# satoken/ractip

Hardware: AMD Instinct MI355X
Metric: sequence-pairs/sec (incl. bp+hp+ap DP; host strings in, thresholded matrices out) at n=500 (higher is better)
Workload: dtype f64; 1 GPU; synthetic random pairs n=500/500, std::mt19937(12345) stream (BASELINE config 3); scoring=CONTRAfold complementary (708 weights)

## Files before the change

### ractip_amd/csrc/ctx.h

```cpp
#pragma once
#include <hip/hip_runtime.h>

#include <cassert>
#include <cstdint>
#include <cstring>
#include <string>
#include <type_traits>
#include <vector>

#include "../../include/ractip_hot.h"
#include "batch.h"
#include "batch_request.h"
#include "local_windows.h"
#include "score_model.h"
#include "lin_model.h"
#include "vienna_model.h"
#include "scale_order.h"
#include "span_fold.h"

struct rh_ctx;

namespace rh::host {

struct DevBuf {
// ... 18 lines not shown
        return hipMemcpy(p, host, cap, hipMemcpyHostToDevice);
    }
};

struct LocalHp {
    LocalDuplex2Plan D;
    int windowed = 0;
    bool valid = false;
    DevBuf hp, logz;
    int tile[2] = {0, 0};
    double ms[2] = {0, 0};
};

struct LinSet {
    LinModel h;
    DevObj<LinModel> d;
    DevObj<double> wT;
};

struct VLinSet {
    VLinModel* h = nullptr;
    DevObj<VLinModel> d;
    ~VLinSet() { delete h; }
};

struct GraphSlot {
    hipGraphExec_t exec = nullptr;
    size_t key = 0;
    int launches = 0, far = 0;
};

struct SweepPlan {
    enum Org { kNone, kStrips, kPairs, kLookahead, kDiagonals, kDxStrip8, kDxSweep4, kDxSweepW };
    enum Far { kFarNone, kFarLds, kFarGather, kFarPacked };
    Org org = kNone;
    int W = 0;
    int BS = 0;
    int filt = 0;
    Far far = kFarNone;
    int far2_from = 0;
    int banded = 0;
    int repack2 = 0;
    const char* fine = "";
    const char* far_name = "";
};

static_assert(std::has_unique_object_representations_v<SweepPlan> && std::has_unique_object_representations_v<McBatch>);
static_assert(sizeof(DxLinBatch) == 4 * sizeof(void*) + 6 * sizeof(int) + 3 * sizeof(size_t) + 16 * sizeof(double), "no padding");

struct McLinArgs {
    McBatch B;
    const LinSet* lin;
    double* logz;
    int* bad;
    SweepPlan plan;
    const int* small_list;
    const int* n_sweep;
    const int* n_short;
    SweepPlan plan_sweep, plan_short;
    int routed, n_small, nmax_sweep, short_count, nmax_short;
    int phase, pin, strip_xcd;
    int f5_pass, f5_jlo;
    int up_w, pad_;
    McLinArgs() { std::memset(this, 0, sizeof *this); }
};

struct McVlinArgs {
// ... 81 lines not shown
    DevObj<DxLinModel> d_dxlin_r[4];
    DxLinModel h_dxlin_r[4];
    std::vector<int> rescaled_dx;
    DxLinBatch dxl = {};
    size_t dxl_layout = 0;
    size_t dx_bytes = 0;
    bool dxtab_log = false;
    int co_seed = 1;
    int dx_strip = 1;
    int dx_quad = 1;
    int dx_w = 4;
    int last_dx_path = 0;
    int far_mfma = 1;
    int lookahead = 2;
    int strip = 3;
    int far2 = -1;
    int strip_w = 8;
    int small_on = 0;
    std::vector<int> small_list;
    DevBuf d_small_list;
    DevBuf d_n_sweep;
    int nmax_sweep = 0;
    DevBuf d_n_short;
    int n_short = 0, nmax_short = 0;
    int strip_filt = 1;
    bool strip_filt_ok = false;
    int co_cut_min = 0, co_cut_max = 0;
    int co_window = 1;
    int acc_final_t = 1;
    int acc_wide = 1;
    int strip_xcd = 1;
    int f5_pass = 1;
    int far_pk = 1;
    int use_graphs = 1;
    GraphSlot g_in, g_out, g_dx;
    int mode = RH_MODE_AUTO;
    int duplex_mode = RH_MODE_INHERIT;
    int lin_w = 4;
    int lin_w_in = 4;
    int lin_bs = 16;
    int last_path = 0;
    bool last_went_log = false;
    SweepPlan plan[3];
    int max_w = 1;
    int region_acc = 0;
    DevBuf d_acc;
    hipEvent_t acc_ev[2] = {nullptr, nullptr};
    bool acc_timed = false;

    int np = 0, ns = 0;
    std::vector<int> pair_seq;
    std::vector<int> pair_seq_dev;
    bool indexed = false;
    bool has_mc = false, has_dx = false, computed = false;
    std::vector<int> n;
    McBatch mc = {};
    DxBatch dx = {};
    DevBuf d_seq;
    DevBuf d_n;
    DevBuf d_pseq;
    DevBuf d_pn;
    DevBuf d_pidx;
    DevBuf d_mctab;
    DevBuf d_corowp;
    DevBuf d_rowp;
    DevBuf d_pk;
// ... 160 lines not shown
```

### ractip_amd/csrc/kernels.h

```cpp
#pragma once
#include <hip/hip_runtime.h>

#include "../../include/ractip_hot.h"
#include "batch.h"
#include "score_model.h"
#include "lin_model.h"
#include "vienna_model.h"

namespace rh {
__global__ void mc_init(McBatch B);
__global__ void mc_inside_diag(McBatch B, const ScoreModel* __restrict__ M, int d, int pin);
__global__ void mc_outside_diag(McBatch B, const ScoreModel* __restrict__ M, int d, int pin);
__global__ void mc_unpaired(McBatch B, int max_w);
struct AccArgs {
    const LinModel* lin;
    const ScoreModel* score;
    double* scratch;
    int max_w, pad_;
};
constexpr int kAccTile = 64, kAccK = 16;
constexpr size_t acc_scratch_doubles(int ld) { return 3 * (size_t)ld * ld + 2 * 31 * (size_t)ld; }
template <int PATH> __global__ void cf_acc_hrows(McBatch B, AccArgs A);
template <int PATH> __global__ void cf_acc_hcols(McBatch B, AccArgs A);
template <int PATH> __global__ void cf_acc_gaps(McBatch B, AccArgs A);
template <int PATH> __global__ void cf_acc_final(McBatch B, AccArgs A);
template <int PATH> __global__ void cf_acc_sbuild(McBatch B, AccArgs A);
template <int PATH> __global__ void cf_acc_seed(McBatch B, AccArgs A);
template <int PATH> __global__ void cf_acc_link(McBatch B, AccArgs A, int flip);
template <int PATH> __global__ void cf_acc_close(McBatch B, AccArgs A, int j, int flip);
__global__ void dx_sweep_diag(DxBatch B, const ScoreModel* __restrict__ M, int t);
__global__ void dx_logz(DxBatch B, const ScoreModel* __restrict__ M);
__global__ void dx_posterior(DxBatch B);
__global__ void dx_hp_clear_rest(DxBatch B);
__global__ void lin_init(McBatch B, const LinModel* __restrict__ L, int* __restrict__ bad);
template <int W, int BS, int MODE> __global__ void lin_inside_diag(McBatch B, const LinModel* __restrict__ L, int d, double lam_d, int pin);
template <int W, int BS> __global__ void lin_outside_diag(McBatch B, const LinModel* __restrict__ L, int d, int pin, int* __restrict__ bad);
template <int W, int BS> __global__ void lin_outside_pair(McBatch B, const LinModel* __restrict__ L, int d, int khi, int pin, int* __restrict__ bad);
template <int BS> __global__ void lin_far_inside(McBatch B, int D);
template <int BS> __global__ void lin_far_outside(McBatch B, int D);
__global__ void lin_far_inside_mfma(McBatch B, int D);
__global__ void lin_far_outside_mfma(McBatch B, int D);
template <int SWEEP> __global__ void lin_pack_tiles(McBatch B, int Dblk, int outside, int banded);
template <int KD, int W, int FILT> __global__ void lin_inside_strip(McBatch B, const LinModel* __restrict__ L, const double* __restrict__ wT, int d0, double lam_d0, int pin);
template <int KD, int W, int FILT> __global__ void lin_outside_strip(McBatch B, const LinModel* __restrict__ L, const double* __restrict__ wT, int d0, int pin, int* __restrict__ bad);
__global__ void lin_f5i_tail(McBatch B, const LinModel* __restrict__ L, int jlo);
__global__ void lin_f5i_pass(McBatch B, const LinModel* __restrict__ L, int jlo);
void launch_lin_small(const McBatch& B, const LinModel* L, const double* wpad, const int* list, int nlist, int* bad, hipStream_t stream);
__global__ void lin_f5o_head(McBatch B, const LinModel* __restrict__ L, int khi, int klo);
__global__ void lin_f5o_pass(McBatch B, const LinModel* __restrict__ L);
__global__ void lin_far_inside_pk(McBatch B, int D, int l2);
__global__ void lin_far_outside_pk(McBatch B, int D, int l2);
__global__ void lin_far2_inside(McBatch B, int D2, int l2);
__global__ void lin_far2_outside(McBatch B, int D2, int l2);
__global__ void lin_finish(McBatch B, const LinModel* __restrict__ L, double* __restrict__ logz, int* __restrict__ bad);
template <int W> __global__ void dxl_sweep(DxLinBatch B, const DxLinModel* __restrict__ L, int step, int groups);
__global__ void dxl_sweep4(DxLinBatch B, const DxLinModel* __restrict__ L, int step, int groups);
__global__ void dxl_strip8(DxLinBatch B, const DxLinModel* __restrict__ L, int step);
template <bool S20> __global__ void dxvl_sweep4(DxLinBatch B, const VLinModel* __restrict__ L, const VDxLin* __restrict__ D, int step);
template <bool S20> __global__ void dxvl_logz_part(DxLinBatch B, const VLinModel* __restrict__ L, const VDxLin* __restrict__ D, double* __restrict__ zpart,
                               int* __restrict__ cpart, int nchunk);
__global__ void dxvl_logz_final(DxLinBatch B, double s, const double* __restrict__ zpart, const int* __restrict__ cpart, int nchunk,
                                double* __restrict__ zbar, double* __restrict__ logz, int* __restrict__ bad);
constexpr int kLzThreads = 256;
size_t dxl_logz_lds_bytes(int lds);
__global__ void dxl_logz_part(DxLinBatch B, const DxLinModel* __restrict__ L, double* __restrict__ zpart, int* __restrict__ cpart, int nchunk);
__global__ void dxl_logz_final(DxLinBatch B, const DxLinModel* __restrict__ L, const double* __restrict__ zpart, const int* __restrict__ cpart, int nchunk,
                               double* __restrict__ zbar, double* __restrict__ logz, int* __restrict__ bad);
__global__ void dxl_posterior(DxLinBatch B, const double* __restrict__ zbar, int* __restrict__ bad);
__global__ void dxv_sweep_diag(DxBatch B, const ViennaDx* __restrict__ V, int t);
__global__ void dxv_logz(DxBatch B, const ViennaDx* __restrict__ V);
__global__ void dxv_posterior(DxBatch B);
__global__ void mcv_init(McBatch B);
__global__ void mcv_inside_diag(McBatch B, const ViennaDx* __restrict__ V, int d, int pin);
__global__ void mcv_outside_diag(McBatch B, const ViennaDx* __restrict__ V, int d, int pin);
__global__ void mcv_acc_prep(McBatch B, const ViennaDx* __restrict__ V);
__global__ void mcv_acc_hscan(McBatch B, int slot);
__global__ void vlin_acc_prep(McBatch B, const VLinModel* __restrict__ L, const double* __restrict__ hplen);
__global__ void vlin_acc_gaps(McBatch B, const VLinModel* __restrict__ L, double* __restrict__ gaps, int ng, int nchunk, double* __restrict__ part);
__global__ void vlin_acc_gsum(McBatch B, double* __restrict__ gaps, const double* __restrict__ part, int ng, int nchunk);
__global__ void vlin_acc_gaps_wide(McBatch B, const VLinModel* __restrict__ L, double* __restrict__ gaps);
__global__ void vlin_acc_final_t(McBatch B, const VLinModel* __restrict__ L, const double* __restrict__ gaps, int max_w);
__global__ void vlin_acc_hsum(McBatch B, int max_w);
__global__ void vlin_acc_gsuf(McBatch B, double* __restrict__ gaps);
__global__ void vlin_acc_final(McBatch B, const VLinModel* __restrict__ L, const double* __restrict__ gaps, int max_w);
// ... 64 lines not shown
```

### ractip_amd/csrc/launch_contrafold.hip

```cpp
#include <hip/hip_runtime.h>

#include <algorithm>
#include <cmath>
#include <cstring>
#include <string>
#include <vector>

#include "ctx.h"
#include "f5_stage.h"
#include "kernels.h"

__global__ void log_finish(rh::McBatch B, double* __restrict__ logz)
{
    const int sq = blockIdx.x * blockDim.x + threadIdx.x;
    if (sq < B.ns) logz[sq] = B.f5i[(size_t)sq * B.ld + B.n[sq]];
}

namespace rh::host {

int launch_mc_log(rh_ctx* c, int pin, const McBatch& B, double* logz_out)
{
    hipLaunchKernelGGL(mc_init, dim3((B.ns + 63) / 64), dim3(64), 0, c->s_mc, B);
    for (int d = 0; d <= B.nmax - 1; d++) {
        const int waves = std::max(B.nmax - 1 - d, 0) + 1;
        KLAUNCH(c, 0, mc_inside_diag, pin ? dim3(B.ns, (waves + 3) / 4) : dim3((waves + 3) / 4, B.ns), dim3(256), c->s_mc, B, c->d_model, d, pin);
        c->n_launch[0]++;
    }
    HIP_TRY(c, hipEventRecord(c->ev[kEvMcInside], c->s_mc));
    for (int d = B.nmax - 2; d >= 0; d--) {
        const int waves = (B.nmax - 1 - d) + 1;
        KLAUNCH(c, 2, mc_outside_diag, pin ? dim3(B.ns, (waves + 3) / 4) : dim3((waves + 3) / 4, B.ns), dim3(256), c->s_mc, B, c->d_model, d, pin);
        c->n_launch[1]++;
    }
    hipLaunchKernelGGL(log_finish, dim3((B.ns + 63) / 64), dim3(64), 0, c->s_mc, B, logz_out);
    hipLaunchKernelGGL(mc_unpaired, dim3((B.nmax + 63) / 64, B.ns), dim3(256), 0, c->s_mc, B, c->max_w);
    return RH_OK;
}

template <int PATH>
static void acc_kernels(const McBatch& B, const AccArgs& A, hipStream_t st)
{
    const int n = B.nmax, ns = B.ns, w = A.max_w;
    hipLaunchKernelGGL(cf_acc_hrows<PATH>, dim3((n + 255) / 256, ns), dim3(256), 0, st, B, A);
// ... 19 lines not shown
    A.lin = lin ? (const LinModel*)lin->d : nullptr;
    A.score = c->d_model;
    A.scratch = c->d_acc.as<double>();
    A.max_w = c->max_w;
    if (timed) {
        for (auto& e : c->acc_ev) if (!e) HIP_TRY(c, hipEventCreate(&e));
        HIP_TRY(c, hipEventRecord(c->acc_ev[0], c->s_mc));
    }
    if (lin) acc_kernels<0>(B, A, c->s_mc);
    else acc_kernels<1>(B, A, c->s_mc);
    HIP_TRY(c, hipGetLastError());
    if (timed) {
        HIP_TRY(c, hipEventRecord(c->acc_ev[1], c->s_mc));
        c->acc_timed = true;
    }
    return RH_OK;
}

using InsideDiagK = void (*)(McBatch, const LinModel*, int, double, int);
struct DiagKernels { int W, BS; Named<InsideDiagK> in; Named<decltype(&lin_outside_diag<4, 16>)> out; };
#define DIAG(W, BS) {W, BS, NAMED(lin_inside_diag<W, BS, 0>), NAMED(lin_outside_diag<W, BS>)}
const DiagKernels kDiag[] = {DIAG(8, 0), DIAG(16, 0), DIAG(4, 16), DIAG(8, 16), DIAG(16, 16), DIAG(8, 32), DIAG(16, 32)};
const Named<InsideDiagK> kInsidePair = NAMED(lin_inside_diag<4, 16, 3>);
const Named<InsideDiagK> kInsideAhead[2] = {NAMED(lin_inside_diag<4, 16, 1>), NAMED(lin_inside_diag<4, 16, 2>)};
struct PairKernels { int W; Named<decltype(&lin_outside_pair<4, 16>)> out; };
const PairKernels kOutsidePair[] = {{4, NAMED(lin_outside_pair<4, 16>)}, {8, NAMED(lin_outside_pair<8, 16>)}};
struct StripKernels { int W, filt; Named<decltype(&lin_inside_strip<8, 4, 0>)> in; Named<decltype(&lin_outside_strip<8, 4, 0>)> out; };
#define STRIP(W, FILT) {W, FILT, NAMED(lin_inside_strip<8, W, FILT>), NAMED(lin_outside_strip<8, W, FILT>)}
const StripKernels kStrip[] = {STRIP(4, 0), STRIP(8, 1), STRIP(8, 0)};
struct LdsKernels { int BS; Named<decltype(&lin_far_inside<16>)> in, out; };
const LdsKernels kLds[] = {{16, NAMED(lin_far_inside<16>), NAMED(lin_far_outside<16>)}, {32, NAMED(lin_far_inside<32>), NAMED(lin_far_outside<32>)}};
const Named<decltype(&lin_far_inside_mfma)> kFarGather[2] = {NAMED(lin_far_inside_mfma), NAMED(lin_far_outside_mfma)};
const Named<decltype(&lin_far_inside_pk)> kFarPacked[2] = {NAMED(lin_far_inside_pk), NAMED(lin_far_outside_pk)};
#undef DIAG
#undef STRIP
static const DiagKernels& diag_kernels(int W, int BS) { return row_of(kDiag, [&](const DiagKernels& r) { return r.W == W && r.BS == BS; }); }
static const PairKernels& pair_kernels(int W) { return row_of(kOutsidePair, [&](const PairKernels& r) { return r.W == W; }); }
static const StripKernels& strip_kernels(int W, int filt) { return row_of(kStrip, [&](const StripKernels& r) { return r.W == W && r.filt == filt; }); }
static const LdsKernels& lds_kernels(int BS) { return row_of(kLds, [&](const LdsKernels& r) { return r.BS == BS; }); }

const char* far_name(SweepPlan::Far far, int BS, int phase)
{
    switch (far) {
        case SweepPlan::kFarLds: return phase == 0 ? lds_kernels(BS).in.name : lds_kernels(BS).out.name;
        case SweepPlan::kFarGather: return kFarGather[phase].name;
        case SweepPlan::kFarPacked: return kFarPacked[phase].name;
        default: return "";
    }
}
void far_products(const rh_ctx* c, int phase, int nmax, bool mfma, SweepPlan* P)
{
    const int from = c->far2 >= 0 ? (c->far2 ? 1 : 0) : 384;
    P->far = P->BS == 0 ? SweepPlan::kFarNone : !mfma ? SweepPlan::kFarLds : c->far_pk ? SweepPlan::kFarPacked : SweepPlan::kFarGather;
    P->far2_from = P->far == SweepPlan::kFarPacked && from > 0 && nmax >= from ? from : 0;
    P->far_name = far_name(P->far, P->BS, phase);
}

void far_inside_after(const SweepPass& S, int done)
{
    rh_ctx* c = S.c;
    const McBatch& B = S.B;
    const int D = S.P.BS ? done / S.P.BS + 1 : 0, last_block = S.last_block(), l2 = S.P.far2_from;
    if (S.P.BS == 0 || done % S.P.BS != 0 || D < 4 || D > last_block) return;
    if (S.P.far == SweepPlan::kFarLds) KLAUNCH(c, 1, (lds_kernels(S.P.BS).in.kern), dim3(last_block - D + 1, B.ns), dim3(256), S.st, B, D);
    else if (S.P.far == SweepPlan::kFarGather) KLAUNCH(c, 1, (kFarGather[0].kern), dim3(last_block - D + 1, B.ns), dim3(256), S.st, B, D);
    else {
        KLAUNCH(c, 1, lin_pack_tiles<0>, dim3(B.nb - (D - 2), B.ns, 2), dim3(256), S.st, B, D - 2, 0, (int)S.P.banded);
        if (l2 && (D + 3) % 4 == 0) {
            const int D2 = (D + 3) / 4, last2 = (B.nmax - 1) / 64;
            if (D2 >= 4 && D2 <= last2) KLAUNCH(c, 1, lin_far2_inside, dim3(last2 - D2 + 1, B.ns), dim3(256), S.st, B, D2, l2);
        }
        KLAUNCH(c, 1, (kFarPacked[0].kern), dim3(last_block - D + 1, B.ns), dim3(256), S.st, B, D, l2);
    }
    c->n_launch[S.k]++;
    c->n_far[S.k]++;
}
void far_outside_before(SweepPass& S, int d)
{
    rh_ctx* c = S.c;
    const McBatch& B = S.B;
    const int D = S.P.BS ? (d + 1) / S.P.BS - 1 : 0, last_block = S.last_block(), l2 = S.P.far2_from;
    if (S.P.BS == 0 || (d + 1) % S.P.BS != 0 || D < 0 || D > last_block) return;
    if (S.P.far == SweepPlan::kFarLds) KLAUNCH(c, 3, (lds_kernels(S.P.BS).out.kern), dim3(last_block - D + 1, B.ns, 2), dim3(256), S.st, B, D);
    else if (S.P.far == SweepPlan::kFarGather) KLAUNCH(c, 3, (kFarGather[1].kern), dim3(last_block - D + 1, B.ns, 2), dim3(256), S.st, B, D);
    else {
        if (D + 2 <= last_block) KLAUNCH(c, 3, lin_pack_tiles<1>, dim3(B.nb - (D + 2), B.ns, 1), dim3(256), S.st, B, D + 2, 1, 0);
        if (l2) {
            const int last2 = (B.nmax - 1) / 64;
            for (; S.far2_next >= 0 && 4 * S.far2_next + 3 >= D; S.far2_next--)
                KLAUNCH(c, 3, lin_far2_outside, dim3(last2 - S.far2_next + 1, B.ns, 2), dim3(256), S.st, B, S.far2_next, l2);
        }
        KLAUNCH(c, 3, (kFarPacked[1].kern), dim3(last_block - D + 1, B.ns, 2), dim3(256), S.st, B, D, l2);
    }
    c->n_launch[S.k]++;
    c->n_far[S.k]++;
}
void far_outside_begin(SweepPass& S, int top)
{
    if (S.P.BS == 0) return;
    rh_ctx* c = S.c;
    const McBatch& B = S.B;
    const int last_block = S.last_block(), banded = S.P.banded;
    if (S.P.far == SweepPlan::kFarPacked) {
        S.far2_next = (B.nmax - 1) / 64;
        if (S.P.repack2 && last_block - 1 > 2) KLAUNCH(c, 3, lin_pack_tiles<1>, dim3(B.nb - 2, B.ns, 2), dim3(256), S.st, B, 2, 0, banded);
        for (int Dblk = std::max(2, last_block - 1); Dblk <= last_block; Dblk++)
            KLAUNCH(c, 3, lin_pack_tiles<1>, dim3(B.nb - Dblk, B.ns, 2), dim3(256), S.st, B, Dblk, 0, banded);
    }
    for (int d = (last_block + 1) * S.P.BS - 1; d > top; d -= S.P.BS) far_outside_before(S, d);
}

SweepPlan plan_mc_lin(const rh_ctx* c, int phase, int nmax)
{
    SweepPlan P;
    const int w = phase == 0 ? c->lin_w_in : c->lin_w;
    P.BS = c->lin_bs == 0 || c->lin_bs == 32 ? c->lin_bs : 16;
    P.W = w == 16 ? 16 : (w == 4 && P.BS == 16 ? 4 : 8);
    const bool all_orgs = P.W == 4 && P.BS == 16, strips_ok = c->far_pk && c->far_mfma && c->lin_bs == 16 && nmax >= kStripMinN;
    const bool strips_on = (c->strip & (phase == 0 ? 1 : 2)) && strips_ok, strips = all_orgs && strips_on;
    const StripKernels& strip = strip_kernels(c->strip_w, c->strip_w == 8 && c->strip_filt && c->strip_filt_ok);
    const DiagKernels& diag = diag_kernels(P.W, P.BS);
    bool mfma = P.BS == 16 && c->far_mfma;
    P.org = SweepPlan::kDiagonals;
    P.fine = phase == 0 ? diag.in.name : diag.out.name;
    if (strips) {
        P.org = SweepPlan::kStrips;
        P.W = strip.W;
        P.filt = strip.filt;
    } else if (phase == 0 && all_orgs && c->lookahead == 2) {
        P.org = SweepPlan::kPairs;
        P.fine = kInsidePair.name;
        mfma = true;
    } else if (phase == 0 && all_orgs && c->lookahead) {
        P.org = SweepPlan::kLookahead;
        P.fine = kInsideAhead[0].name;
    } else if (phase == 1 && mfma && (P.W == 4 || P.W == 8) && c->lookahead == 2) {
        P.org = SweepPlan::kPairs;
        P.fine = pair_kernels(P.W).out.name;
    }
    far_products(c, phase, nmax, mfma, &P);
// ... 171 lines not shown
```

### ractip_amd/csrc/mccaskill_far.hip

```cpp
#include <hip/hip_runtime.h>

#include "batch.h"
#include "lin_model.h"
#include "kernels.h"

namespace rh {

static_assert((int)VL_FM1 == (int)L_FM1 && (int)VL_FM == (int)L_FM && (int)VL_FM2O == (int)L_FM2O && (int)VL_FM2F == (int)L_FM2F &&
                  (int)VL_FMOF == (int)L_FMOF && (int)VL_FM1OF == (int)L_FM1OF,
              "LinTable and VLinTable disagree on a slot of the block products: FM1, FM, FM2O, FM2F, FMOF, FM1OF");

namespace {

__device__ __forceinline__ double cellv(const double* __restrict__ T, int ld, int n, int x, int y)
{
    return (x >= 1 && x <= y && y <= n - 1) ? T[(size_t)(y - x) * ld + x] : 0.0;
}

template <int BS, bool TR>
__device__ __forceinline__ void load_chunk(double (*dst)[BS + 1], const double* __restrict__ T, int ld, int n, int x0, int y0)
{
    const int u = threadIdx.x % BS;
    constexpr int DPP = 256 / BS;
    for (int dd = threadIdx.x / BS; dd < 2 * BS - 1; dd += DPP) {
        const int v = u + dd - (BS - 1);
        if (v >= 0 && v < BS) {
            const double val = cellv(T, ld, n, x0 + u, y0 + v);
            if (TR) dst[v][u] = val; else dst[u][v] = val;
        }
    }
}

template <int BS>
struct Acc {
    static constexpr int R = BS / 16;
    double c[R][R];
    __device__ __forceinline__ void zero()
// ... 158 lines not shown
__global__ __launch_bounds__(256) void lin_far_outside_mfma(McBatch B, int D)
{
    __shared__ double A[4][16][17], Bm[4][16][17], red[4][256];
    const int sq = blockIdx.y;
    const int n = B.n[sq];
    const int I = blockIdx.x, J = I + D;
    if (J * 16 > n - 1) return;
    const int w = threadIdx.x >> 6;
    const int ld = B.ld;
    double* __restrict__ tab = B.tab + (size_t)sq * B.seq_stride;
    const double* __restrict__ fm1 = tab + (size_t)L_FM1 * B.tab_stride;
    const double* __restrict__ fm = tab + (size_t)L_FM * B.tab_stride;
    const double* __restrict__ fm2o = tab + (size_t)L_FM2O * B.tab_stride;
    d4 acc = {0.0, 0.0, 0.0, 0.0};
    if (blockIdx.z == 0) {
        for (int K = w; K <= I - 2; K += 4) {
            load_chunk16_wave<true>(A[w], fm1, ld, n, K * 16, I * 16);
            load_chunk16_wave<false>(Bm[w], fm2o, ld, n, K * 16, J * 16);
            acc = mfma_chunk(A[w], Bm[w], acc);
        }
        reduce_store(red, acc, tab + (size_t)L_FMOF * B.tab_stride, ld, n, I * 16, J * 16);
    } else {
        const int last = (n - 1) / 16;
        for (int K = J + 2 + w; K <= last; K += 4) {
            load_chunk16_wave<false>(A[w], fm2o, ld, n, I * 16, K * 16);
            load_chunk16_wave<true>(Bm[w], fm, ld, n, J * 16, K * 16);
            acc = mfma_chunk(A[w], Bm[w], acc);
        }
        reduce_store(red, acc, tab + (size_t)L_FM1OF * B.tab_stride, ld, n, I * 16, J * 16);
    }
}

enum PkCopy { PK_FM1_A = 0, PK_FM1_B, PK_FM_A, PK_FM_B, PK_FM2O_A, PK_FM2O_B };
__device__ __forceinline__ size_t pk_tile(int nb, int P, int Q) { return ((size_t)P * nb - (size_t)P * (P - 1) / 2 + (Q - P)) * 256; }

template <int SWEEP>
__global__ __launch_bounds__(256) void lin_pack_tiles(McBatch B, int Dblk, int outside, int banded)
{
    __shared__ double T[16][17];
    const int sq = blockIdx.y;
    const int n = B.n[sq];
    const int P = blockIdx.x, Q = P + Dblk;
    if (Q >= B.nb || Q * 16 > n - 1) return;
    const int slot = outside ? L_FM2O : (blockIdx.z == 0 ? L_FM1 : L_FM);
    const int copy = outside ? PK_FM2O_A : (blockIdx.z == 0 ? PK_FM1_A : PK_FM_A);
    const double* __restrict__ src = B.tab + (size_t)sq * B.seq_stride + (size_t)slot * B.tab_stride;
    {
        const int u = threadIdx.x & 15;
#pragma unroll
        for (int pass = 0; pass < 2; pass++) {
            const int v = u + (threadIdx.x >> 4) + 16 * pass - 15;
            if (v >= 0 && v < 16) T[u][v] = (banded && !outside && Dblk == 2 && v < u) ? 0.0 : cellv(src, B.ld, n, P * 16 + u, Q * 16 + v);
        }
    }
    __syncthreads();
    double* __restrict__ dst = B.pk + ((size_t)sq * kPkCopies + copy) * B.pk_stride + pk_tile(B.nb, P, Q);
    const int s = threadIdx.x & 3, l = threadIdx.x >> 2, r = l & 15, q = l >> 4;
    dst[threadIdx.x] = T[r][4 * s + q];
    dst[B.pk_stride + threadIdx.x] = T[4 * s + q][r];
}

__device__ __forceinline__ d4 mfma4(d4 a, d4 b, d4 acc)
{
#pragma unroll
    for (int s = 0; s < 4; s++) acc = __builtin_amdgcn_mfma_f64_16x16x4f64(a[s], b[s], acc, 0, 0, 0);
    return acc;
}

template <class TA, class TB>
__device__ __forceinline__ d4 pk_loop(const double* __restrict__ pa, const double* __restrict__ pb, int k_lo, int k_hi, TA ta, TB tb,
                                      d4 acc = d4{0.0, 0.0, 0.0, 0.0})
{
    const int w = threadIdx.x >> 6, lane = threadIdx.x & 63;
    int K = k_lo + w;
    for (; K + 4 <= k_hi; K += 8) {
        const d4 a0 = *(const d4*)(pa + ta(K) + lane * 4), b0 = *(const d4*)(pb + tb(K) + lane * 4);
        const d4 a1 = *(const d4*)(pa + ta(K + 4) + lane * 4), b1 = *(const d4*)(pb + tb(K + 4) + lane * 4);
        acc = mfma4(a0, b0, acc);
        acc = mfma4(a1, b1, acc);
    }
    if (K <= k_hi) {
        const d4 a0 = *(const d4*)(pa + ta(K) + lane * 4), b0 = *(const d4*)(pb + tb(K) + lane * 4);
        acc = mfma4(a0, b0, acc);
    }
    return acc;
}


__device__ __forceinline__ bool one_strand_tile(const McBatch& B, int sq, bool inside, int lo_i, int hi_j)
{
    if (!B.cut || (inside && !B.seeded)) return false;
    const int cut = B.cut[sq];
    return cut > 0 && (hi_j + 1 <= cut || lo_i > cut);
}

__global__ __launch_bounds__(256) void lin_far_inside_pk(McBatch B, int D, int l2)
{
    __shared__ double red[4][256];
    const int sq = blockIdx.y;
    const int n = B.n[sq];
    const int I = blockIdx.x, J = I + D;
    if (J * 16 > n - 1) return;
    if (one_strand_tile(B, sq, true, I * 16, J * 16 + 15)) return;
    const int nb = B.nb;
    const double* __restrict__ pk = B.pk + (size_t)sq * kPkCopies * B.pk_stride;
    const auto ta = [=](int K) { return pk_tile(nb, I, K); };
    const auto tb = [=](int K) { return pk_tile(nb, K, J); };
    const int I2 = I >> 2, J2 = J >> 2;
    const bool two = l2 > 0 && n >= l2 && J2 - I2 >= 4;
    d4 acc = pk_loop(pk + PK_FM1_A * B.pk_stride, pk + PK_FM_B * B.pk_stride, I + 2, two ? 4 * (I2 + 2) - 1 : J - 2, ta, tb);
    if (two) acc = pk_loop(pk + PK_FM1_A * B.pk_stride, pk + PK_FM_B * B.pk_stride, 4 * (J2 - 1), J - 2, ta, tb, acc);
    reduce_store(red, acc, B.tab + (size_t)sq * B.seq_stride + (size_t)L_FM2F * B.tab_stride, B.ld, n, I * 16, J * 16, two);
}

__global__ __launch_bounds__(256) void lin_far_outside_pk(McBatch B, int D, int l2)
{
    __shared__ double red[4][256];
    const int sq = blockIdx.y;
    const int n = B.n[sq];
    const int I = blockIdx.x, J = I + D;
    if (J * 16 > n - 1) return;
    if (one_strand_tile(B, sq, false, I * 16, J * 16 + 15)) return;
    const int nb = B.nb;
    const double* __restrict__ pk = B.pk + (size_t)sq * kPkCopies * B.pk_stride;
    double* __restrict__ tab = B.tab + (size_t)sq * B.seq_stride;
    const int I2 = I >> 2, J2 = J >> 2, last = (n - 1) / 16;
    if (blockIdx.z == 0) {
        const bool two = l2 > 0 && n >= l2 && I2 >= 2;
        const d4 acc = pk_loop(pk + PK_FM1_B * B.pk_stride, pk + PK_FM2O_B * B.pk_stride, two ? 4 * (I2 - 1) : 0, I - 2,
                               [=](int K) { return pk_tile(nb, K, I); }, [=](int K) { return pk_tile(nb, K, J); });
        reduce_store(red, acc, tab + (size_t)L_FMOF * B.tab_stride, B.ld, n, I * 16, J * 16, two);
    } else {
        const bool two = l2 > 0 && n >= l2 && 4 * (J2 + 2) <= last;
        const d4 acc = pk_loop(pk + PK_FM2O_A * B.pk_stride, pk + PK_FM_A * B.pk_stride, J + 2, two ? 4 * (J2 + 2) - 1 : last,
                               [=](int K) { return pk_tile(nb, I, K); }, [=](int K) { return pk_tile(nb, J, K); });
        reduce_store(red, acc, tab + (size_t)L_FM1OF * B.tab_stride, B.ld, n, I * 16, J * 16, two);
    }
}

struct Acc4 { d4 c[2][2]; };
__device__ __forceinline__ void store_quadrant(const Acc4& A, double* __restrict__ T, int ld, int n, int I2, int J2)
{
    const int w = threadIdx.x >> 6, lane = threadIdx.x & 63;
#pragma unroll
    for (int a = 0; a < 2; a++)
#pragma unroll
        for (int b = 0; b < 2; b++) {
            const int i0 = (4 * I2 + 2 * (w >> 1) + a) * 16, j0 = (4 * J2 + 2 * (w & 1) + b) * 16;
#pragma unroll
            for (int r = 0; r < 4; r++) {
                const int i = i0 + (lane >> 4) + 4 * r, j = j0 + (lane & 15);
                if (i >= 1 && i <= j && j <= n - 1) T[(size_t)(j - i) * ld + i] = A.c[a][b][r];
            }
        }
}
template <class TA, class TB>
__device__ __forceinline__ void far2_loop(Acc4& A, const double* __restrict__ pa, const double* __restrict__ pb, int k_lo, int k_hi, TA ta, TB tb)
{
    const int lane = threadIdx.x & 63;
    if (k_lo > k_hi) return;
    d4 a0 = *(const d4*)(pa + ta(0, k_lo) + lane * 4), a1 = *(const d4*)(pa + ta(1, k_lo) + lane * 4);
    d4 b0 = *(const d4*)(pb + tb(k_lo, 0) + lane * 4), b1 = *(const d4*)(pb + tb(k_lo, 1) + lane * 4);
    for (int K = k_lo; K <= k_hi; K++) {
        const int Kn = K < k_hi ? K + 1 : K;
        const d4 na0 = *(const d4*)(pa + ta(0, Kn) + lane * 4), na1 = *(const d4*)(pa + ta(1, Kn) + lane * 4);
        const d4 nb0 = *(const d4*)(pb + tb(Kn, 0) + lane * 4), nb1 = *(const d4*)(pb + tb(Kn, 1) + lane * 4);
        A.c[0][0] = mfma4(a0, b0, A.c[0][0]);
        A.c[0][1] = mfma4(a0, b1, A.c[0][1]);
        A.c[1][0] = mfma4(a1, b0, A.c[1][0]);
        A.c[1][1] = mfma4(a1, b1, A.c[1][1]);
        a0 = na0; a1 = na1; b0 = nb0; b1 = nb1;
    }
}

__global__ __launch_bounds__(256) void lin_far2_inside(McBatch B, int D2, int l2)
{
    const int sq = blockIdx.y;
    const int n = B.n[sq];
    if (n < l2) return;
    const int I2 = blockIdx.x, J2 = I2 + D2;
    if (J2 * 64 > n - 1) return;
    if (one_strand_tile(B, sq, true, I2 * 64, J2 * 64 + 63)) return;
    const int nb = B.nb, w = threadIdx.x >> 6;
    const int Ia = 4 * I2 + 2 * (w >> 1), Jb = 4 * J2 + 2 * (w & 1);
    const double* __restrict__ pk = B.pk + (size_t)sq * kPkCopies * B.pk_stride;
    Acc4 A;
#pragma unroll
    for (int a = 0; a < 2; a++)
#pragma unroll
        for (int b = 0; b < 2; b++) A.c[a][b] = d4{0.0, 0.0, 0.0, 0.0};
    far2_loop(A, pk + PK_FM1_A * B.pk_stride, pk + PK_FM_B * B.pk_stride, 4 * (I2 + 2), 4 * (J2 - 1) - 1,
              [=](int a, int K) { return pk_tile(nb, Ia + a, K); }, [=](int K, int b) { return pk_tile(nb, K, Jb + b < nb ? Jb + b : nb - 1); });
    store_quadrant(A, B.tab + (size_t)sq * B.seq_stride + (size_t)L_FM2F * B.tab_stride, B.ld, n, I2, J2);
}

__global__ __launch_bounds__(256) void lin_far2_outside(McBatch B, int D2, int l2)
{
    const int sq = blockIdx.y;
    const int n = B.n[sq];
// ... 36 lines not shown
```

### ractip_amd/csrc/rh_api.hip

```cpp
#include <hip/hip_runtime.h>

#include <dlfcn.h>

#include <algorithm>
#include <cstdarg>
#include <cstdio>
#include <cstdlib>
#include <cstring>
#include <string>
#include <vector>

#include "ctx.h"
#include "kernels.h"

using namespace rh;
using namespace rh::host;

__global__ void collect_logz(const double* __restrict__ mc_logz, const int* __restrict__ idx, DxBatch D, double* __restrict__ out)
{
    const int p = blockIdx.x * blockDim.x + threadIdx.x;
    if (p >= D.np) return;
    out[3 * p + 0] = mc_logz[idx[2 * p]];
    out[3 * p + 1] = mc_logz[idx[2 * p + 1]];
    out[3 * p + 2] = D.logz[p];
// ... 56 lines not shown
    HIP_TRY(c, hipMemcpy(out, c->d_up.as<const double>() + (size_t)sq * c->mc.ld * c->max_w, sizeof(double) * c->n[sq] * c->max_w,
                         hipMemcpyDeviceToHost));
    return RH_OK;
}
int fetch_logz(rh_ctx* c, int sq, double* out)
{
    HIP_TRY(c, hipMemcpy(out, c->d_mclogz.as<const double>() + sq, sizeof(double), hipMemcpyDeviceToHost));
    return RH_OK;
}
int fetch_hp(rh_ctx* c, int p, double* out, double* logz)
{
    const int n1 = c->n[seq_of(c, p, 0)], n2 = c->n[seq_of(c, p, 1)];
    if (out)
        HIP_TRY(c, hipMemcpy2D(out, sizeof(double) * (n2 + 1), c->d_hp.as<const double>() + (size_t)p * c->dx.tab_stride,
                               sizeof(double) * c->dx.ldd, sizeof(double) * (n2 + 1), n1 + 1, hipMemcpyDeviceToHost));
    if (logz) HIP_TRY(c, hipMemcpy(logz, c->d_logz.as<const double>() + p, sizeof(double), hipMemcpyDeviceToHost));
    return RH_OK;
}

enum EnvKind { ENV_INT, ENV_FLAG , ENV_NOT , ENV_4OR8 , ENV_DOUBLE };
struct EnvSwitch {
    const char* name;
    EnvKind kind;
    int Ctx::*field;
    double Ctx::*dfield = nullptr;
};
const EnvSwitch kEnvSwitches[] = {
    {"RH_LIN_W", ENV_INT, &Ctx::lin_w},        {"RH_LIN_W", ENV_INT, &Ctx::lin_w_in},
    {"RH_LIN_W_IN", ENV_INT, &Ctx::lin_w_in},
    {"RH_LIN_BS", ENV_INT, &Ctx::lin_bs},
    {"RH_NO_GRAPH", ENV_NOT, &Ctx::use_graphs},
    {"RH_FAR_MFMA", ENV_FLAG, &Ctx::far_mfma},
    {"RH_FAR_PK", ENV_FLAG, &Ctx::far_pk},
    {"RH_LOOKAHEAD", ENV_INT, &Ctx::lookahead},
    {"RH_STRIP", ENV_INT, &Ctx::strip},
    {"RH_STRIP_W", ENV_4OR8, &Ctx::strip_w},
    {"RH_STRIP_FILT", ENV_FLAG, &Ctx::strip_filt},
    {"RH_SMALL", ENV_FLAG, &Ctx::small_on},
    {"RH_FAR2", ENV_INT, &Ctx::far2},
    {"RH_STRIP_XCD", ENV_INT, &Ctx::strip_xcd},
    {"RH_F5_PASS", ENV_FLAG, &Ctx::f5_pass},
    {"RH_ACC_WIDE", ENV_INT, &Ctx::acc_wide},
    {"RH_ACC_FINAL_T", ENV_INT, &Ctx::acc_final_t},
    {"RH_CO_WINDOW", ENV_INT, &Ctx::co_window},
    {"RH_SCALE_LADDER", ENV_INT, &Ctx::scale_ladder},
    {"RH_SCALE_MEMORY", ENV_INT, &Ctx::scale_memory},
    {"RH_PAIR_HELPER", ENV_INT, &Ctx::pair_helper},
    {"RH_CO_SEED", ENV_INT, &Ctx::co_seed},
    {"RH_DX_W", ENV_INT, &Ctx::dx_w},
    {"RH_DX_QUAD", ENV_FLAG, &Ctx::dx_quad},
    {"RH_DX_STRIP", ENV_INT, &Ctx::dx_strip},
    {"RH_VDX_S", ENV_DOUBLE, nullptr, &Ctx::vdx_s},
};

}

extern "C" {

static rh_ctx* create_ctx(int device, int model, const char* param_file, const char* defaults_file, int use_bl, int semantics);

rh_ctx* rh_create(int device, int model, const char* param_file) { return create_ctx(device, model, param_file, nullptr, 1, 0); }
rh_ctx* rh_create_vienna(int device, const char* defaults_file, int use_bl_param, const char* param_file, int semantics)
{
    return create_ctx(device, RH_MODEL_VIENNA_BL, param_file, defaults_file, use_bl_param, semantics);
}
int rh_vienna_semantics(const rh_ctx* c) { return c ? c->vienna_sem : RH_ERR_ARG; }
// ... 590 lines not shown
```

Before: 12580 pairs/s.

## Compute far tile products one tile per wave and batch tile packing in runs

```diff
diff --git a/ractip_amd/csrc/ctx.h b/ractip_amd/csrc/ctx.h
--- a/ractip_amd/csrc/ctx.h
+++ b/ractip_amd/csrc/ctx.h
@@ -74,7 +74,8 @@
 
 struct SweepPlan {
     enum Org { kNone, kStrips, kPairs, kLookahead, kDiagonals, kDxStrip8, kDxSweep4, kDxSweepW };
-    enum Far { kFarNone, kFarLds, kFarGather, kFarPacked };
+    enum Far { kFarNone, kFarLds, kFarGather, kFarPacked, kFarPacked4 };
+    bool packed() const { return far == kFarPacked || far == kFarPacked4; }
     Org org = kNone;
     int W = 0;
     int BS = 0;
@@ -222,6 +223,7 @@
     int strip_xcd = 1;
     int f5_pass = 1;
     int far_pk = 1;
+    int far_wave = 1;
     int use_graphs = 1;
     GraphSlot g_in, g_out, g_dx;
     int mode = RH_MODE_AUTO;
diff --git a/ractip_amd/csrc/kernels.h b/ractip_amd/csrc/kernels.h
--- a/ractip_amd/csrc/kernels.h
+++ b/ractip_amd/csrc/kernels.h
@@ -50,6 +50,8 @@
 __global__ void lin_f5o_pass(McBatch B, const LinModel* __restrict__ L);
 __global__ void lin_far_inside_pk(McBatch B, int D, int l2);
 __global__ void lin_far_outside_pk(McBatch B, int D, int l2);
+__global__ void lin_far_inside_pk4(McBatch B, int D, int l2);
+__global__ void lin_far_outside_pk4(McBatch B, int D, int l2);
 __global__ void lin_far2_inside(McBatch B, int D2, int l2);
 __global__ void lin_far2_outside(McBatch B, int D2, int l2);
 __global__ void lin_finish(McBatch B, const LinModel* __restrict__ L, double* __restrict__ logz, int* __restrict__ bad);
diff --git a/ractip_amd/csrc/launch_contrafold.hip b/ractip_amd/csrc/launch_contrafold.hip
--- a/ractip_amd/csrc/launch_contrafold.hip
+++ b/ractip_amd/csrc/launch_contrafold.hip
@@ -9,6 +9,7 @@
 #include "ctx.h"
 #include "f5_stage.h"
 #include "kernels.h"
+#include "pk_layout.h"
 
 __global__ void log_finish(rh::McBatch B, double* __restrict__ logz)
 {
@@ -94,6 +95,7 @@
 const LdsKernels kLds[] = {{16, NAMED(lin_far_inside<16>), NAMED(lin_far_outside<16>)}, {32, NAMED(lin_far_inside<32>), NAMED(lin_far_outside<32>)}};
 const Named<decltype(&lin_far_inside_mfma)> kFarGather[2] = {NAMED(lin_far_inside_mfma), NAMED(lin_far_outside_mfma)};
 const Named<decltype(&lin_far_inside_pk)> kFarPacked[2] = {NAMED(lin_far_inside_pk), NAMED(lin_far_outside_pk)};
+const Named<decltype(&lin_far_inside_pk)> kFarPacked4[2] = {NAMED(lin_far_inside_pk4), NAMED(lin_far_outside_pk4)};
 #undef DIAG
 #undef STRIP
 static const DiagKernels& diag_kernels(int W, int BS) { return row_of(kDiag, [&](const DiagKernels& r) { return r.W == W && r.BS == BS; }); }
@@ -107,17 +109,26 @@
         case SweepPlan::kFarLds: return phase == 0 ? lds_kernels(BS).in.name : lds_kernels(BS).out.name;
         case SweepPlan::kFarGather: return kFarGather[phase].name;
         case SweepPlan::kFarPacked: return kFarPacked[phase].name;
+        case SweepPlan::kFarPacked4: return kFarPacked4[phase].name;
         default: return "";
     }
 }
 void far_products(const rh_ctx* c, int phase, int nmax, bool mfma, SweepPlan* P)
 {
     const int from = c->far2 >= 0 ? (c->far2 ? 1 : 0) : 384;
-    P->far = P->BS == 0 ? SweepPlan::kFarNone : !mfma ? SweepPlan::kFarLds : c->far_pk ? SweepPlan::kFarPacked : SweepPlan::kFarGather;
-    P->far2_from = P->far == SweepPlan::kFarPacked && from > 0 && nmax >= from ? from : 0;
+    P->far = P->BS == 0 ? SweepPlan::kFarNone : !mfma ? SweepPlan::kFarLds : !c->far_pk ? SweepPlan::kFarGather : c->far_wave ? SweepPlan::kFarPacked : SweepPlan::kFarPacked4;
+    P->far2_from = P->packed() && from > 0 && nmax >= from ? from : 0;
     P->far_name = far_name(P->far, P->BS, phase);
 }
 
+static void far_packed_launch(const SweepPass& S, int phase, int D, int l2)
+{
+    rh_ctx* c = S.c;
+    const bool wave = S.P.far == SweepPlan::kFarPacked;
+    const int tiles = S.last_block() - D + 1;
+    const dim3 grid(wave ? (tiles + 3) / 4 : tiles, S.B.ns, phase == 0 ? 1 : 2);
+    KLAUNCH(c, phase == 0 ? 1 : 3, ((wave ? kFarPacked : kFarPacked4)[phase].kern), grid, dim3(256), S.st, S.B, D, l2);
+}
 void far_inside_after(const SweepPass& S, int done)
 {
     rh_ctx* c = S.c;
@@ -127,12 +138,12 @@
     if (S.P.far == SweepPlan::kFarLds) KLAUNCH(c, 1, (lds_kernels(S.P.BS).in.kern), dim3(last_block - D + 1, B.ns), dim3(256), S.st, B, D);
     else if (S.P.far == SweepPlan::kFarGather) KLAUNCH(c, 1, (kFarGather[0].kern), dim3(last_block - D + 1, B.ns), dim3(256), S.st, B, D);
     else {
-        KLAUNCH(c, 1, lin_pack_tiles<0>, dim3(B.nb - (D - 2), B.ns, 2), dim3(256), S.st, B, D - 2, 0, (int)S.P.banded);
+        KLAUNCH(c, 1, lin_pack_tiles<0>, dim3(pk_run_groups(B.nb - (D - 2)), B.ns, 2), dim3(256), S.st, B, D - 2, 0, (int)S.P.banded);
         if (l2 && (D + 3) % 4 == 0) {
             const int D2 = (D + 3) / 4, last2 = (B.nmax - 1) / 64;
             if (D2 >= 4 && D2 <= last2) KLAUNCH(c, 1, lin_far2_inside, dim3(last2 - D2 + 1, B.ns), dim3(256), S.st, B, D2, l2);
         }
-        KLAUNCH(c, 1, (kFarPacked[0].kern), dim3(last_block - D + 1, B.ns), dim3(256), S.st, B, D, l2);
+        far_packed_launch(S, 0, D, l2);
     }
     c->n_launch[S.k]++;
     c->n_far[S.k]++;
@@ -146,13 +157,13 @@
     if (S.P.far == SweepPlan::kFarLds) KLAUNCH(c, 3, (lds_kernels(S.P.BS).out.kern), dim3(last_block - D + 1, B.ns, 2), dim3(256), S.st, B, D);
     else if (S.P.far == SweepPlan::kFarGather) KLAUNCH(c, 3, (kFarGather[1].kern), dim3(last_block - D + 1, B.ns, 2), dim3(256), S.st, B, D);
     else {
-        if (D + 2 <= last_block) KLAUNCH(c, 3, lin_pack_tiles<1>, dim3(B.nb - (D + 2), B.ns, 1), dim3(256), S.st, B, D + 2, 1, 0);
+        if (D + 2 <= last_block) KLAUNCH(c, 3, lin_pack_tiles<1>, dim3(pk_run_groups(B.nb - (D + 2)), B.ns, 1), dim3(256), S.st, B, D + 2, 1, 0);
         if (l2) {
             const int last2 = (B.nmax - 1) / 64;
             for (; S.far2_next >= 0 && 4 * S.far2_next + 3 >= D; S.far2_next--)
                 KLAUNCH(c, 3, lin_far2_outside, dim3(last2 - S.far2_next + 1, B.ns, 2), dim3(256), S.st, B, S.far2_next, l2);
         }
-        KLAUNCH(c, 3, (kFarPacked[1].kern), dim3(last_block - D + 1, B.ns, 2), dim3(256), S.st, B, D, l2);
+        far_packed_launch(S, 1, D, l2);
     }
     c->n_launch[S.k]++;
     c->n_far[S.k]++;
@@ -163,11 +174,11 @@
     rh_ctx* c = S.c;
     const McBatch& B = S.B;
     const int last_block = S.last_block(), banded = S.P.banded;
-    if (S.P.far == SweepPlan::kFarPacked) {
+    if (S.P.packed()) {
         S.far2_next = (B.nmax - 1) / 64;
-        if (S.P.repack2 && last_block - 1 > 2) KLAUNCH(c, 3, lin_pack_tiles<1>, dim3(B.nb - 2, B.ns, 2), dim3(256), S.st, B, 2, 0, banded);
+        if (S.P.repack2 && last_block - 1 > 2) KLAUNCH(c, 3, lin_pack_tiles<1>, dim3(pk_run_groups(B.nb - 2), B.ns, 2), dim3(256), S.st, B, 2, 0, banded);
         for (int Dblk = std::max(2, last_block - 1); Dblk <= last_block; Dblk++)
-            KLAUNCH(c, 3, lin_pack_tiles<1>, dim3(B.nb - Dblk, B.ns, 2), dim3(256), S.st, B, Dblk, 0, banded);
+            KLAUNCH(c, 3, lin_pack_tiles<1>, dim3(pk_run_groups(B.nb - Dblk), B.ns, 2), dim3(256), S.st, B, Dblk, 0, banded);
     }
     for (int d = (last_block + 1) * S.P.BS - 1; d > top; d -= S.P.BS) far_outside_before(S, d);
 }
diff --git a/ractip_amd/csrc/mccaskill_far.hip b/ractip_amd/csrc/mccaskill_far.hip
--- a/ractip_amd/csrc/mccaskill_far.hip
+++ b/ractip_amd/csrc/mccaskill_far.hip
@@ -3,6 +3,7 @@
 #include "batch.h"
 #include "lin_model.h"
 #include "kernels.h"
+#include "pk_layout.h"
 
 namespace rh {
 
@@ -227,32 +228,44 @@
 }
 
 enum PkCopy { PK_FM1_A = 0, PK_FM1_B, PK_FM_A, PK_FM_B, PK_FM2O_A, PK_FM2O_B };
-__device__ __forceinline__ size_t pk_tile(int nb, int P, int Q) { return ((size_t)P * nb - (size_t)P * (P - 1) / 2 + (Q - P)) * 256; }
+__device__ __forceinline__ size_t pk_tile(int nb, int P, int Q) { return ((size_t)P * nb - (size_t)P * (P - 1) / 2 + (Q - P)) * kPkTile; }
+typedef double d2 __attribute__((ext_vector_type(2)));
+__device__ __forceinline__ d4 pk_frag(const double* __restrict__ tile, int lane)
+{
+    const d2 lo = *(const d2*)(tile + pk_half_offset(lane, 0)), hi = *(const d2*)(tile + pk_half_offset(lane, 1));
+    return d4{lo.x, lo.y, hi.x, hi.y};
+}
 
 template <int SWEEP>
 __global__ __launch_bounds__(256) void lin_pack_tiles(McBatch B, int Dblk, int outside, int banded)
 {
-    __shared__ double T[16][17];
-    const int sq = blockIdx.y;
-    const int n = B.n[sq];
-    const int P = blockIdx.x, Q = P + Dblk;
-    if (Q >= B.nb || Q * 16 > n - 1) return;
+    __shared__ double T[kPkRun][16][17];
+    const int sq = blockIdx.y;
+    const int n = B.n[sq];
+    const int P0 = blockIdx.x * kPkRun, R = pk_run_tiles(B.nb, n, Dblk, P0);
+    if (R <= 0) return;
     const int slot = outside ? L_FM2O : (blockIdx.z == 0 ? L_FM1 : L_FM);
     const int copy = outside ? PK_FM2O_A : (blockIdx.z == 0 ? PK_FM1_A : PK_FM_A);
     const double* __restrict__ src = B.tab + (size_t)sq * B.seq_stride + (size_t)slot * B.tab_stride;
-    {
-        const int u = threadIdx.x & 15;
-#pragma unroll
-        for (int pass = 0; pass < 2; pass++) {
-            const int v = u + (threadIdx.x >> 4) + 16 * pass - 15;
-            if (v >= 0 && v < 16) T[u][v] = (banded && !outside && Dblk == 2 && v < u) ? 0.0 : cellv(src, B.ld, n, P * 16 + u, Q * 16 + v);
-        }
+    const bool mask = banded && !outside && Dblk == 2;
+    double val[kPkRunPasses];
+#pragma unroll
+    for (int q = 0; q < kPkRunPasses; q++) {
+        const PkRunItem it = pk_run_item(threadIdx.x, q, R);
+        val[q] = (it.in && !(mask && it.v < it.u)) ? cellv(src, B.ld, n, (P0 + it.p) * 16 + it.u, (P0 + it.p + Dblk) * 16 + it.v) : 0.0;
+    }
+#pragma unroll
+    for (int q = 0; q < kPkRunPasses; q++) {
+        const PkRunItem it = pk_run_item(threadIdx.x, q, R);
+        if (it.in) T[it.p][it.u][it.v] = val[q];
     }
     __syncthreads();
-    double* __restrict__ dst = B.pk + ((size_t)sq * kPkCopies + copy) * B.pk_stride + pk_tile(B.nb, P, Q);
-    const int s = threadIdx.x & 3, l = threadIdx.x >> 2, r = l & 15, q = l >> 4;
-    dst[threadIdx.x] = T[r][4 * s + q];
-    dst[B.pk_stride + threadIdx.x] = T[4 * s + q][r];
+    const int u = pk_store_u(threadIdx.x), v = pk_store_v(threadIdx.x);
+    for (int p = 0; p < R; p++) {
+        double* __restrict__ dst = B.pk + ((size_t)sq * kPkCopies + copy) * B.pk_stride + pk_tile(B.nb, P0 + p, P0 + p + Dblk);
+        dst[threadIdx.x] = T[p][u][v];
+        dst[B.pk_stride + threadIdx.x] = T[p][v][u];
+    }
 }
 
 __device__ __forceinline__ d4 mfma4(d4 a, d4 b, d4 acc)
@@ -262,23 +275,43 @@
     return acc;
 }
 
-template <class TA, class TB>
-__device__ __forceinline__ d4 pk_loop(const double* __restrict__ pa, const double* __restrict__ pb, int k_lo, int k_hi, TA ta, TB tb,
-                                      d4 acc = d4{0.0, 0.0, 0.0, 0.0})
+struct PkTiles {
+    const double* __restrict__ p;
+    int nb, fixed, row;
+    __device__ __forceinline__ const double* operator()(int K) const { return p + (row ? pk_tile(nb, fixed, K) : pk_tile(nb, K, fixed)); }
+};
+
+__device__ __forceinline__ d4 pk_loop(int k_lo, int k_hi, PkTiles ta, PkTiles tb, d4 acc)
 {
     const int w = threadIdx.x >> 6, lane = threadIdx.x & 63;
     int K = k_lo + w;
     for (; K + 4 <= k_hi; K += 8) {
-        const d4 a0 = *(const d4*)(pa + ta(K) + lane * 4), b0 = *(const d4*)(pb + tb(K) + lane * 4);
-        const d4 a1 = *(const d4*)(pa + ta(K + 4) + lane * 4), b1 = *(const d4*)(pb + tb(K + 4) + lane * 4);
+        const d4 a0 = pk_frag(ta(K), lane), b0 = pk_frag(tb(K), lane);
+        const d4 a1 = pk_frag(ta(K + 4), lane), b1 = pk_frag(tb(K + 4), lane);
         acc = mfma4(a0, b0, acc);
         acc = mfma4(a1, b1, acc);
     }
     if (K <= k_hi) {
-        const d4 a0 = *(const d4*)(pa + ta(K) + lane * 4), b0 = *(const d4*)(pb + tb(K) + lane * 4);
+        const d4 a0 = pk_frag(ta(K), lane), b0 = pk_frag(tb(K), lane);
         acc = mfma4(a0, b0, acc);
     }
     return acc;
+}
+
+__device__ __forceinline__ void wave_loop(d4 (&acc)[4], int k_lo, int k_hi, PkTiles ta, PkTiles tb)
+{
+    const int lane = threadIdx.x & 63;
+    d4 fa[4], fb[4];
+#pragma unroll
+    for (int w = 0; w < 4; w++)
+        if (k_lo + w <= k_hi) { fa[w] = pk_frag(ta(k_lo + w), lane); fb[w] = pk_frag(tb(k_lo + w), lane); }
+    for (int K = k_lo; K <= k_hi; K += 4) {
+#pragma unroll
+        for (int w = 0; w < 4; w++) {
+            if (K + w <= k_hi) acc[w] = mfma4(fa[w], fb[w], acc[w]);
+            if (K + w + 4 <= k_hi) { fa[w] = pk_frag(ta(K + w + 4), lane); fb[w] = pk_frag(tb(K + w + 4), lane); }
+        }
+    }
 }
 
 
@@ -289,49 +322,107 @@
     return cut > 0 && (hi_j + 1 <= cut || lo_i > cut);
 }
 
-__global__ __launch_bounds__(256) void lin_far_inside_pk(McBatch B, int D, int l2)
-{
-    __shared__ double red[4][256];
-    const int sq = blockIdx.y;
-    const int n = B.n[sq];
-    const int I = blockIdx.x, J = I + D;
+struct FarProduct {
+    PkTiles ta, tb;
+    int lo1, hi1, lo2, hi2;
+    double* __restrict__ T;
+    int i0, j0, rmw;
+};
+
+template <bool WAVE>
+__device__ __forceinline__ void far_product(const FarProduct& P, int ld, int n)
+{
+    const d4 zero = {0.0, 0.0, 0.0, 0.0};
+    if constexpr (WAVE) {
+        const int lane = threadIdx.x & 63;
+        double* t[4];
+        bool in[4];
+        double old[4];
+#pragma unroll
+        for (int r = 0; r < 4; r++) {
+            const int i = P.i0 + (lane >> 4) + 4 * r, j = P.j0 + (lane & 15);
+            in[r] = i >= 1 && i <= j && j <= n - 1;
+            t[r] = P.T + (size_t)(j - i) * ld + i;
+            old[r] = P.rmw && in[r] ? *t[r] : 0.0;
+        }
+        d4 acc[4] = {zero, zero, zero, zero};
+        wave_loop(acc, P.lo1, P.hi1, P.ta, P.tb);
+        wave_loop(acc, P.lo2, P.hi2, P.ta, P.tb);
+        const d4 v = ((acc[0] + acc[1]) + acc[2]) + acc[3];
+#pragma unroll
+        for (int r = 0; r < 4; r++)
+            if (in[r]) *t[r] = P.rmw ? old[r] + v[r] : v[r];
+    } else {
+        __shared__ double red[4][256];
+        d4 acc = pk_loop(P.lo1, P.hi1, P.ta, P.tb, zero);
+        acc = pk_loop(P.lo2, P.hi2, P.ta, P.tb, acc);
+        reduce_store(red, acc, P.T, ld, n, P.i0, P.j0, P.rmw);
+    }
+}
+
+template <bool WAVE>
+__device__ __forceinline__ int far_tile_index()
+{
+    return WAVE ? 4 * (int)blockIdx.x + __builtin_amdgcn_readfirstlane((int)(threadIdx.x >> 6)) : (int)blockIdx.x;
+}
+
+template <bool WAVE>
+__device__ __forceinline__ void far_inside_tile(const McBatch& B, int D, int l2)
+{
+    const int sq = blockIdx.y;
+    const int n = B.n[sq];
+    const int I = far_tile_index<WAVE>(), J = I + D;
     if (J * 16 > n - 1) return;
     if (one_strand_tile(B, sq, true, I * 16, J * 16 + 15)) return;
-    const int nb = B.nb;
     const double* __restrict__ pk = B.pk + (size_t)sq * kPkCopies * B.pk_stride;
-    const auto ta = [=](int K) { return pk_tile(nb, I, K); };
-    const auto tb = [=](int K) { return pk_tile(nb, K, J); };
     const int I2 = I >> 2, J2 = J >> 2;
     const bool two = l2 > 0 && n >= l2 && J2 - I2 >= 4;
-    d4 acc = pk_loop(pk + PK_FM1_A * B.pk_stride, pk + PK_FM_B * B.pk_stride, I + 2, two ? 4 * (I2 + 2) - 1 : J - 2, ta, tb);
-    if (two) acc = pk_loop(pk + PK_FM1_A * B.pk_stride, pk + PK_FM_B * B.pk_stride, 4 * (J2 - 1), J - 2, ta, tb, acc);
-    reduce_store(red, acc, B.tab + (size_t)sq * B.seq_stride + (size_t)L_FM2F * B.tab_stride, B.ld, n, I * 16, J * 16, two);
-}
-
-__global__ __launch_bounds__(256) void lin_far_outside_pk(McBatch B, int D, int l2)
-{
-    __shared__ double red[4][256];
-    const int sq = blockIdx.y;
-    const int n = B.n[sq];
-    const int I = blockIdx.x, J = I + D;
+    FarProduct P;
+    P.ta = PkTiles{pk + PK_FM1_A * B.pk_stride, B.nb, I, 1};
+    P.tb = PkTiles{pk + PK_FM_B * B.pk_stride, B.nb, J, 0};
+    P.lo1 = I + 2; P.hi1 = two ? 4 * (I2 + 2) - 1 : J - 2;
+    P.lo2 = two ? 4 * (J2 - 1) : 1; P.hi2 = two ? J - 2 : 0;
+    P.T = B.tab + (size_t)sq * B.seq_stride + (size_t)L_FM2F * B.tab_stride;
+    P.i0 = I * 16; P.j0 = J * 16; P.rmw = two;
+    far_product<WAVE>(P, B.ld, n);
+}
+
+template <bool WAVE>
+__device__ __forceinline__ void far_outside_tile(const McBatch& B, int D, int l2)
+{
+    const int sq = blockIdx.y;
+    const int n = B.n[sq];
+    const int I = far_tile_index<WAVE>(), J = I + D;
     if (J * 16 > n - 1) return;
     if (one_strand_tile(B, sq, false, I * 16, J * 16 + 15)) return;
-    const int nb = B.nb;
     const double* __restrict__ pk = B.pk + (size_t)sq * kPkCopies * B.pk_stride;
     double* __restrict__ tab = B.tab + (size_t)sq * B.seq_stride;
     const int I2 = I >> 2, J2 = J >> 2, last = (n - 1) / 16;
+    FarProduct P;
+    P.lo2 = 1; P.hi2 = 0;
+    P.i0 = I * 16; P.j0 = J * 16;
     if (blockIdx.z == 0) {
         const bool two = l2 > 0 && n >= l2 && I2 >= 2;
-        const d4 acc = pk_loop(pk + PK_FM1_B * B.pk_stride, pk + PK_FM2O_B * B.pk_stride, two ? 4 * (I2 - 1) : 0, I - 2,
-                               [=](int K) { return pk_tile(nb, K, I); }, [=](int K) { return pk_tile(nb, K, J); });
-        reduce_store(red, acc, tab + (size_t)L_FMOF * B.tab_stride, B.ld, n, I * 16, J * 16, two);
+        P.ta = PkTiles{pk + PK_FM1_B * B.pk_stride, B.nb, I, 0};
+        P.tb = PkTiles{pk + PK_FM2O_B * B.pk_stride, B.nb, J, 0};
+        P.lo1 = two ? 4 * (I2 - 1) : 0; P.hi1 = I - 2;
+        P.T = tab + (size_t)L_FMOF * B.tab_stride;
+        P.rmw = two;
     } else {
         const bool two = l2 > 0 && n >= l2 && 4 * (J2 + 2) <= last;
-        const d4 acc = pk_loop(pk + PK_FM2O_A * B.pk_stride, pk + PK_FM_A * B.pk_stride, J + 2, two ? 4 * (J2 + 2) - 1 : last,
-                               [=](int K) { return pk_tile(nb, I, K); }, [=](int K) { return pk_tile(nb, J, K); });
-        reduce_store(red, acc, tab + (size_t)L_FM1OF * B.tab_stride, B.ld, n, I * 16, J * 16, two);
-    }
-}
+        P.ta = PkTiles{pk + PK_FM2O_A * B.pk_stride, B.nb, I, 1};
+        P.tb = PkTiles{pk + PK_FM_A * B.pk_stride, B.nb, J, 1};
+        P.lo1 = J + 2; P.hi1 = two ? 4 * (J2 + 2) - 1 : last;
+        P.T = tab + (size_t)L_FM1OF * B.tab_stride;
+        P.rmw = two;
+    }
+    far_product<WAVE>(P, B.ld, n);
+}
+
+__global__ __launch_bounds__(256) void lin_far_inside_pk(McBatch B, int D, int l2) { far_inside_tile<true>(B, D, l2); }
+__global__ __launch_bounds__(256) void lin_far_outside_pk(McBatch B, int D, int l2) { far_outside_tile<true>(B, D, l2); }
+__global__ __launch_bounds__(256) void lin_far_inside_pk4(McBatch B, int D, int l2) { far_inside_tile<false>(B, D, l2); }
+__global__ __launch_bounds__(256) void lin_far_outside_pk4(McBatch B, int D, int l2) { far_outside_tile<false>(B, D, l2); }
 
 struct Acc4 { d4 c[2][2]; };
 __device__ __forceinline__ void store_quadrant(const Acc4& A, double* __restrict__ T, int ld, int n, int I2, int J2)
@@ -354,12 +445,12 @@
 {
     const int lane = threadIdx.x & 63;
     if (k_lo > k_hi) return;
-    d4 a0 = *(const d4*)(pa + ta(0, k_lo) + lane * 4), a1 = *(const d4*)(pa + ta(1, k_lo) + lane * 4);
-    d4 b0 = *(const d4*)(pb + tb(k_lo, 0) + lane * 4), b1 = *(const d4*)(pb + tb(k_lo, 1) + lane * 4);
+    d4 a0 = pk_frag(pa + ta(0, k_lo), lane), a1 = pk_frag(pa + ta(1, k_lo), lane);
+    d4 b0 = pk_frag(pb + tb(k_lo, 0), lane), b1 = pk_frag(pb + tb(k_lo, 1), lane);
     for (int K = k_lo; K <= k_hi; K++) {
         const int Kn = K < k_hi ? K + 1 : K;
-        const d4 na0 = *(const d4*)(pa + ta(0, Kn) + lane * 4), na1 = *(const d4*)(pa + ta(1, Kn) + lane * 4);
-        const d4 nb0 = *(const d4*)(pb + tb(Kn, 0) + lane * 4), nb1 = *(const d4*)(pb + tb(Kn, 1) + lane * 4);
+        const d4 na0 = pk_frag(pa + ta(0, Kn), lane), na1 = pk_frag(pa + ta(1, Kn), lane);
+        const d4 nb0 = pk_frag(pb + tb(Kn, 0), lane), nb1 = pk_frag(pb + tb(Kn, 1), lane);
         A.c[0][0] = mfma4(a0, b0, A.c[0][0]);
         A.c[0][1] = mfma4(a0, b1, A.c[0][1]);
         A.c[1][0] = mfma4(a1, b0, A.c[1][0]);
diff --git a/ractip_amd/csrc/pk_layout.h b/ractip_amd/csrc/pk_layout.h
--- /dev/null
+++ b/ractip_amd/csrc/pk_layout.h
@@ -0,0 +1,39 @@
+#pragma once
+
+#if defined(__HIPCC__) || defined(__CUDACC__)
+#define PK_HD __host__ __device__
+#else
+#define PK_HD
+#endif
+
+namespace rh {
+
+constexpr int kPkTile = 256;
+constexpr int kPkHalf = 128;
+
+PK_HD constexpr int pk_reg_index(int l, int s) { return (s >> 1) * kPkHalf + 2 * l + (s & 1); }
+PK_HD constexpr int pk_half_offset(int l, int h) { return h * kPkHalf + 2 * l; }
+PK_HD constexpr int pk_la_index(int u, int v) { return pk_reg_index(u + 16 * (v & 3), v >> 2); }
+PK_HD constexpr int pk_lb_index(int u, int v) { return pk_la_index(v, u); }
+
+PK_HD constexpr int pk_store_lane(int t) { return (t & (kPkHalf - 1)) >> 1; }
+PK_HD constexpr int pk_store_reg(int t) { return 2 * (t >> 7) + (t & 1); }
+PK_HD constexpr int pk_store_u(int t) { return pk_store_lane(t) & 15; }
+PK_HD constexpr int pk_store_v(int t) { return 4 * pk_store_reg(t) + (pk_store_lane(t) >> 4); }
+
+constexpr int kPkRun = 8;
+constexpr int kPkRunPasses = 16;
+struct PkRunItem { int dd, p, u, v; bool in; };
+PK_HD constexpr PkRunItem pk_run_item(int t, int q, int R)
+{
+    const int item = t + 256 * q, dd = item >> 7, pos = item & 127, p = pos >> 4, u = pos & 15, v = u + dd - 15;
+    return PkRunItem{dd, p, u, v, dd < 31 && p < R && v >= 0 && v < 16};
+}
+PK_HD constexpr int pk_run_tiles(int nb, int n, int Dblk, int P0)
+{
+    const int lastQ = (n - 1) / 16 < nb - 1 ? (n - 1) / 16 : nb - 1, R = lastQ - Dblk - P0 + 1;
+    return R < 0 ? 0 : R < kPkRun ? R : kPkRun;
+}
+PK_HD constexpr int pk_run_groups(int tiles) { return (tiles + kPkRun - 1) / kPkRun; }
+
+}
diff --git a/ractip_amd/csrc/rh_api.hip b/ractip_amd/csrc/rh_api.hip
--- a/ractip_amd/csrc/rh_api.hip
+++ b/ractip_amd/csrc/rh_api.hip
@@ -112,6 +112,7 @@
     {"RH_NO_GRAPH", ENV_NOT, &Ctx::use_graphs},
     {"RH_FAR_MFMA", ENV_FLAG, &Ctx::far_mfma},
     {"RH_FAR_PK", ENV_FLAG, &Ctx::far_pk},
+    {"RH_FAR_WAVE", ENV_FLAG, &Ctx::far_wave},
     {"RH_LOOKAHEAD", ENV_INT, &Ctx::lookahead},
     {"RH_STRIP", ENV_INT, &Ctx::strip},
     {"RH_STRIP_W", ENV_4OR8, &Ctx::strip_w},
```

After: 12860 pairs/s, median of 6. +2.3%, better.
